# alv-around/mini-stark

Hardware: AMD Instinct MI355X
Metric: stark_proofs_per_s (higher is better)
Workload: dtype u64; 1 GPU; Fibonacci AIR, Goldilocks, 2^20 trace rows, blowup 8, 20 security bits (w=3, c=6, rounds=23, ood_queries=1, fri_queries=2); a step = 8 independent proofs in flight per GPU

## Files before the change

### mini-stark_amd/csrc/ctx.hpp

```cpp
#pragma once
#include "../../include/ministark.h"

#include <cstdarg>
#include <cstdio>
#include <cstdlib>
#include <map>
#include <new>
#include <string>
#include <type_traits>
#include <vector>

#include "field.hpp"
#include "merkle.hpp"
#include "ntt.hpp"
#include "poly.hpp"

namespace msctx {

struct DevBuf {
  void* p = nullptr; size_t cap = 0;
  int ensure(size_t bytes) {
    if (bytes <= cap) return 0;
    if (p) msrt::free_dev(p);
    p = nullptr; cap = 0;
// ... 251 lines not shown
  int finish_sharded_tree(TreeShape& ts, DevBuf& nodes, size_t Mloc);
  template <int EL>
  int tree_build_sharded_contiguous(const T* base, size_t col_stride, size_t row_stride, size_t limb_stride, u32 width, TreeShape& ts, DevBuf& nodes);
  int read_root(const DevBuf& nodes, const TreeShape& ts, u8* root);

  size_t N = 0, w = 0, L = 0, blowup = 0;
  int npolys = 0; size_t polys_cap = 0;
  struct Lin { std::vector<u64> s; std::vector<int> idx; };
  std::vector<Lin> poly_lin;
  std::vector<char> poly_mat; int lazy_lin = 1;
  void expand(int i, T scale, std::map<int, T>& acc) const {
    const Lin& li = poly_lin[i];
    if (li.idx.empty()) { auto it = acc.find(i); if (it == acc.end()) acc[i] = scale; else it->second = F::add(it->second, scale); return; }
    for (size_t t = 0; t < li.idx.size(); t++) expand(li.idx[t], F::mul(scale, F::from_u64(li.s[t] % F::P)), acc);
  }
  int materialize(int i);
  bool have_trace = false, have_polys = false, have_lde = false, have_validity = false;
  DevBuf d_trace[2], d_polys, d_coef, d_lde, d_trace_nodes, d_lde_nodes, d_io, d_partials, d_small;
  TreeShape trace_ts, lde_ts;
  size_t lde_c = 0;

  struct Round { DevBuf poly, cw, nodes; size_t cap = 0, ncoef = 0, D = 0; TreeShape ts; size_t m = 0;
                 bool dist = false, local_store = false; size_t S = 0;
                 bool base_cw = false;  };
  size_t shard_gather_chunk = 0;
  int shard_dist = 1;
  int proof_root_only = 0;
  const T* lpoly(const Round* r) const { return r->local_store ? r->poly.template as<T>() : r->poly.template as<T>() + (size_t)sh_rank * r->S; }
  size_t lstride(const Round* r) const { return r->local_store ? r->S : r->cap; }
  size_t lcount(const Round* r, size_t n) const { const size_t lo = (size_t)sh_rank * r->S; return n <= lo ? 0 : (n - lo < r->S ? n - lo : r->S); }
  size_t dist_chunk(size_t D) const {
    if (!sh_on || !shard_dist || !fri_blowup || !shardable(D / 2)) return 0;
    const size_t den = fri_blowup * (size_t)sh_world;
    if (D % den) return 0;
    const size_t S = D / den;
    return (S >= 2 && !(S & 1)) ? S : 0;
  }
  DevBuf d_carry, d_lq, d_pack, d_fullpoly;
  std::vector<Round*> rounds; size_t nrounds_done = 0, fri_rounds = 0, fri_blowup = 0;
  bool have_deep = false; XE cur_z; XE cur_B[2];
  DevBuf d_folded, d_sh, d_blob, d_tabs, d_targets, d_idx, d_deg, d_ovf;
  size_t blob_size = 0;

  int ensure_polys(size_t count);

  int init(int dev, u32 flags);
  ~Ctx() {
// ... 89 lines not shown
  template <int EC>
  int eval_views(const T* base, size_t poly_stride, size_t limb_stride, size_t kstride, const size_t* off, const size_t* count, int npoly, const XE& z, T* dst);
  template <int EC, int ITEMS>
  int eval_views_i(const T* base, size_t poly_stride, size_t limb_stride, size_t kstride, const size_t* off, const size_t* count, int npoly, const XE& z, T* dst, size_t maxc);
  static bool load_ext(const u64* v, XE* out) { for (int l = 0; l < E; l++) { if (v[l] >= F::P) return false; out->c[l] = F::from_u64(v[l]); } return true; }

  int shard_combine_launch(size_t off, size_t rank_stride, u32 n, const XE& zstep, T* out);
  bool dist_eval() const { return sh_on && shard_dist && N >= shard_min_leaves && N >= (size_t)sh_world * 2; }
  std::vector<int> eval_set() const { std::vector<int> ev; for (int i = 0; i < npolys; i++) if (poly_mat[i]) ev.push_back(i); ev.push_back(npolys); return ev; }
  int eval_finish(int q, const std::vector<int>& ev, u64* out);
  int eval_ext_sharded(const u64* z, int q, u64* out);

  int eval_ext(const u64* z, int q, u64* out) override;

  Round* round_slot(size_t i) { while (rounds.size() <= i) rounds.push_back(new Round()); return rounds[i]; }
  int round_commit(Round* r, size_t ncoef_in, int nonzero_limbs = E, const Round* prev = nullptr, const XE* alpha = nullptr);
  int degree_launch(const T* poly, size_t limb_stride, size_t n, unsigned long long** dres_out);
  int read_degree_and_root(const T* poly, size_t limb_stride, size_t n, Round* r, size_t* ncoef, u8* root);
  int fri_begin(size_t blowup_, size_t nrounds, u8* root0) override;
  int fri_deep(const u64* z, u64* B) override;

  typedef mspoly::SHJob<F, E> SHJ;
  typedef mspoly::SuffixHornerKernel<F, E> SHK;
  struct SHPlan { int nl; std::vector<SHJ> agg; std::vector<SHJ> fin; bool has_top_agg = false; SHJ top_agg; size_t P = 0; bool dist = false; };
  static size_t sh_scratch_elems(size_t m) {
    const size_t BS = mspoly::SH_BS;
    size_t tot = 0, cur = m;
    for (;;) { size_t nb = cur ? (cur + BS - 1) / BS : 1; tot += 2 * nb * E; if (nb <= 1) break; cur = nb; }
    return tot;
  }
  SHPlan sh_plan(const T* in, size_t in_limb_stride, size_t in_off, size_t in_stride, size_t m, const XE& z,
                 void* out, bool out_u64, size_t out_limb_stride, size_t out_off, size_t out_stride, T* h0, T* scratch,
                 const T* ext_carry = nullptr, T* top_agg = nullptr, bool out_h0 = false);
  static XE carry_scale(const XE& z, size_t m, size_t P) { return e_pow<F, E>(e_inv<F>(z), (u64)(P - m)); }
  int sh_launch_inline(const SHJ& j, int final_mode);
  int sh_launch_table(const SHJ* d_jobs, size_t njobs, size_t maxnb, int final_mode);
  int shard_carry_table(const mspoly::CarryJob<F, E>* d_jobs, size_t njobs);
  int suffix_horner(const T* in, size_t in_limb_stride, size_t in_off, size_t in_stride, size_t m, const XE& z,
                    T* out, size_t out_limb_stride, size_t out_off, size_t out_stride, T* h0);

  int gather_poly(const T* local, size_t S, size_t count, T* dst, size_t dst_stride);
  int fold_dist(Round* pr, Round* nr, const XE& a, size_t* nq_coef_out);
  int fri_fold_commit(const u64* alpha, u8* root) override;
  size_t fri_tail_max = (size_t)1 << 15;
  int fri_overlap = 0;
  msrt::Stream* side_stream = nullptr; msrt::Event* ev_side = nullptr; bool side_pending = false;
  struct StreamScope { Ctx* c; msrt::Stream* keep; StreamScope(Ctx* c_, msrt::Stream* s) : c(c_), keep(c_->stream) { c->stream = s; } ~StreamScope() { c->stream = keep; } };
  int join_side() { if (side_pending) { side_pending = false; CK(msrt::stream_wait_event(stream, ev_side)); } return 0; }
  int fri_tail_round(Round* pr, Round* nr, const XE& a, bool* done);
  template <class DG> int fri_tail_round_t(Round* pr, Round* nr, const XE& a, bool* done);
  int fri_round_info(int r, u64* ncoef, u64* D) override;
  int fri_round_poly_read(int r, u64* out) override;
  int fri_round_codeword_read(int r, u64* out) override;

  bool blob_external = false;
  int fri_query(const u64* betas, int nq, u8* ext_out, size_t ext_cap, size_t* ext_len) override;
  struct QueryPlan {
    typedef mspoly::CarryJob<F, E> CJ; typedef mspoly::FindJob<F, E> FJ; typedef msmerkle::PathJob<F, E> PJ; typedef msmerkle::ShardPathJob<F, E> SPJ;
    size_t W = 0; int nq = 0; size_t pos = 0; u8* blob = nullptr;
    T* d_h0 = nullptr; T* d_tg = nullptr; unsigned long long* d_ix = nullptr;
    std::vector<size_t> rec_off, path_off; std::vector<u64> qlen; std::vector<T> x1h;
    std::vector<std::vector<SHJ>> tables; std::vector<int> table_mode, table_part; size_t n_agg_tables = 0;
    std::vector<CJ> carry_jobs; bool any_dist = false;
    std::vector<msmerkle::CopyJob> unp; std::vector<size_t> unp_first, unp_cnt, chunk_c0, chunk_len;
    std::vector<FJ> fjobs; std::vector<PJ> pjobs; std::vector<SPJ> sjobs; std::vector<msmerkle::CopyJob> cjobs; size_t stage_bytes = 0;
    std::vector<size_t> toff; size_t off_f = 0, off_p = 0, off_sp = 0, off_cj = 0, off_rec = 0, off_ql = 0, off_x1 = 0, off_cr = 0, off_un = 0; const u8* dt = nullptr;
  };
  int query_layout(QueryPlan& q, int nq);
  int query_build(QueryPlan& q, const u64* betas);
  int query_scans(QueryPlan& q);
  int query_shard_assembly(QueryPlan& q);
  int query_openings(QueryPlan& q);
  size_t fri_proof_size() const override { return blob_size; }
  int fri_proof_read(u8* out) override;
  msrt::Stream* copy_stream = nullptr; msrt::Event* ev_blob = nullptr; msrt::Event* ev_copy = nullptr; bool copy_pending = false;
  int readback_sdma = 2, sdma_gpu = -1, sdma_state = 0 , last_io_engine = 0;
  msrt::Sdma::Signal sdma_sig{0}, sdma_up_sig{0}; bool sdma_pending = false; int upload_sdma = 1;
  u8* readback_dst = nullptr; size_t readback_bytes = 0;
  double sdma_timeout_s = 20.0;
  bool sdma_ready();
  int poison(const char* what);
  int io_engine() const override { return last_io_engine; }
  int fri_proof_read_async(u8* out) override;
  int fri_proof_wait() override;
  struct Upload { const u64* src = nullptr; size_t N = 0, w = 0; int slot = 0; bool pending = false; } up;
  int trace_slot = 0;
  int trace_upload_async(const u64* trace, size_t N_, size_t w_) override;
  int trace_to_device(const u64* trace, const u64** dsrc);
  int upload_wait(const char* what);

  int merkle_commit(const u64* leafs, size_t leaf_num, int ext, size_t lpn, size_t ic, u8* nodes_out, size_t cap, size_t* nn, u8* root) override;
  template <int EL>
  int merkle_prove_t(const u64* leafs, size_t leaf_num, size_t lpn, const u64* leaf, u8* out, size_t cap, size_t* len);
// ... 10 lines not shown
```

### mini-stark_amd/csrc/fri_commit.cpp

```cpp
#include "ctx.hpp"
#include "fri_tail.hpp"

namespace msctx {

template <class F>
int Ctx<F>::round_commit(Round* r, size_t ncoef_in, int nonzero_limbs, const Round* prev, const XE* alpha) {
  if (ctz64(r->D) > F::TWO_ADICITY) return fail(MS_ERR_SHAPE, "FRI domain larger than the field's two-adicity");
  RQ(tree_shape(r->D, 2, 2, &r->ts));
  r->m = 0;
  r->base_cw = false;
  {
    const bool shard_next = shardable(r->D / 2);
    bool z_outside_base = false;
    for (int l = 1; l < E; l++) z_outside_base = z_outside_base || cur_z.c[l] != 0;
    if (prev && fri_pointwise && z_outside_base && prev->D == 2 * r->D && prev->ts.sharded == shard_next) {
      Plan* pl;
      RQ(get_plan(ctz64(prev->D), 0, false, &pl));
      const size_t W = (size_t)sh_world;
      const size_t m_out = shard_next ? r->D / (2 * W) : r->D;
      const size_t local = shard_next ? 2 * m_out : r->D;
      if (shard_next) r->m = m_out;
      if (r->cw.ensure(local * E * sizeof(T))) return fail(MS_ERR_NOMEM, "codeword");
      const size_t total = m_out * (shard_next ? 2 : 1);
      const XE c = e_add<F, E>(cur_B[0], e_mul<F>(cur_B[1], *alpha));
// ... 101 lines not shown

template <class F>
int Ctx<F>::fri_begin(size_t blowup_, size_t nrounds, u8* root0) {
  if (!have_validity) return fail(MS_ERR_STATE, "fri_begin before mix");
  if (!root0 || nrounds < 1 || !blowup_) return fail(MS_ERR_ARG, "fri_begin");
  nrounds_done = 0; have_deep = false; blob_size = 0;
  fri_rounds = nrounds; fri_blowup = blowup_;
  if (!d_deg.p && d_deg.ensure(256)) return fail(MS_ERR_NOMEM, "degree word");
  CK(msrt::memset_dev(d_deg.p, 0, 256, stream));
  Round* r = round_slot(0);
  const size_t VL = validity_len;
  r->cap = VL;
  if (r->poly.ensure(VL * E * sizeof(T))) return fail(MS_ERR_NOMEM, "round poly");
  CK(msrt::memset_dev(r->poly.p, 0, VL * E * sizeof(T), stream));
  CK(msrt::d2d(r->poly.p, d_polys.as<T>() + (size_t)npolys * N, VL * sizeof(T), stream));
  size_t nc;
  if (validity_len_host) nc = validity_ncoef;
  else RQ(read_degree_and_root(r->poly.template as<T>(), r->cap, VL, nullptr, &nc, nullptr));
  r->ncoef = nc;
  const size_t deg = nc ? nc - 1 : 0;
  size_t dsize = (deg + 1) * blowup_;
  size_t D = 1; while (D < dsize) D <<= 1;
  r->D = D;
  r->S = dist_chunk(D); r->dist = r->S != 0; r->local_store = false;
  RQ(round_commit(r, nc, 1));
  RQ(read_root(r->nodes, r->ts, root0));
  nrounds_done = 1;
  return MS_OK;
}

template <class F>
int Ctx<F>::fri_deep(const u64* z, u64* B) {
  if (nrounds_done == 0 || nrounds_done >= fri_rounds) return fail(MS_ERR_STATE, "fri_deep out of order");
  if (!z || !B) return fail(MS_ERR_ARG, "fri_deep");
  if (!load_ext(z, &cur_z)) return fail(MS_ERR_ARG, "z not canonical");
  Round* r = rounds[nrounds_done - 1];
  size_t off[2] = {0, 1}, cnt[2] = {(r->ncoef + 1) / 2, r->ncoef / 2};
  T* dst = reinterpret_cast<T*>(pinned);
  if (r->dist) {
    const size_t lc = lcount(r, r->ncoef);
    cnt[0] = (lc + 1) / 2; cnt[1] = lc / 2;
    { PartScope part(this); RQ((eval_views<E>(lpoly(r), 0, lstride(r), 2, off, cnt, 2, cur_z, reinterpret_cast<T*>(xs)))); }
    RQ(exchange(MS_XCHG_ALL_GATHER, 2 * E * sizeof(T)));
    RQ(shard_combine_launch(0, 2 * E, 2, e_pow<F, E>(cur_z, (u64)(r->S / 2)), dst));
  } else
  { arm_next_eval = true; RQ((eval_views<E>(r->poly.template as<T>(), 0, r->cap, 2, off, cnt, 2, cur_z, dst))); }
// ... 138 lines not shown
  }
  *nq_coef_out = nq_coef;
  return 0;
}

template <class F>
int Ctx<F>::fri_tail_round(Round* pr, Round* nr, const XE& a, bool* done) {
  if (digest == MS_DIGEST_KECCAK256) return fri_tail_round_t<msmerkle::Keccak256Kernels>(pr, nr, a, done);
  if (digest == MS_DIGEST_SHA3_256) return fri_tail_round_t<msmerkle::Sha3_256Kernels>(pr, nr, a, done);
  if (digest == MS_DIGEST_BLAKE3) return fri_tail_round_t<msmerkle::Blake3Kernels>(pr, nr, a, done);
  return digest == MS_DIGEST_BLAKE2S256 ? fri_tail_round_t<msmerkle::Blake2sKernels>(pr, nr, a, done) : fri_tail_round_t<msmerkle::Sha256Kernels>(pr, nr, a, done);
}
template <class F> template <class DG>
int Ctx<F>::fri_tail_round_t(Round* pr, Round* nr, const XE& a, bool* done) {
  *done = false;
  const size_t n = pr->ncoef, m = (n + 1) / 2, Dn = nr->D, M = Dn / 2;
  bool z_outside_base = false;
  for (int l = 1; l < E; l++) z_outside_base = z_outside_base || cur_z.c[l] != 0;
  if (!fri_tail_max || pr->D > fri_tail_max || pr->dist || pr->ts.sharded || shardable(M) || !fri_pointwise || !z_outside_base || m > (size_t)mspoly::SH_BS || M < 1) return 0;
  typedef msfri::FriTailKernel<F, E, DG> TK;
  if (M > (size_t)TK::WG_GROUPS << TK::TreeK::MAX_LEVELS) return 0;
  if (ctz64(Dn) > F::TWO_ADICITY) return fail(MS_ERR_SHAPE, "FRI domain larger than the field's two-adicity");
  RQ(tree_shape(Dn, 2, 2, &nr->ts));
  nr->m = 0; nr->base_cw = false;
  if (nr->poly.ensure(nr->cap * E * sizeof(T)) || d_folded.ensure((m + 1) * E * sizeof(T)) || nr->cw.ensure(Dn * E * sizeof(T)) || nr->nodes.ensure(nr->ts.nodes * 32) ||
      d_sh.ensure(sh_scratch_elems(m) * sizeof(T)))
    return fail(MS_ERR_NOMEM, "fused FRI round");
  Plan* pl;
  RQ(get_plan(ctz64(pr->D), 0, false, &pl));
  typename TK::Params tp;
  memset(&tp, 0, sizeof tp);
  tp.do_coef = m >= 2 ? 1 : 0;
  tp.fold = typename TK::FoldK::Params{pr->poly.template as<T>(), pr->cap, n, d_folded.as<T>(), m, a, nullptr};
  if (tp.do_coef) {
    SHPlan sp = sh_plan(d_folded.as<T>(), m, 0, 1, m, cur_z, nr->poly.template as<T>(), false, nr->cap, 0, 1, nullptr, d_sh.as<T>());
    if (sp.nl != 1) return fail(MS_ERR_STATE, "fused FRI round: scan of more than one block");
    tp.scan.jobs = nullptr; tp.scan.inline_job = sp.fin[0]; tp.scan.final_mode = 1;
  }
  unsigned long long* dres = d_deg.as<unsigned long long>();
  tp.deg = typename TK::DegK::Params{nr->poly.template as<T>(), nr->cap, m >= 2 ? m - 1 : 0, dres, 0};
  const size_t per = M < (size_t)TK::WG_GROUPS ? M : (size_t)TK::WG_GROUPS, G = M / per;
  tp.G = (u32)G;
  const XE c = e_add<F, E>(cur_B[0], e_mul<F>(cur_B[1], a));
  tp.eval.src = pr->cw.template as<T>(); tp.eval.src_limb_stride = pr->D; tp.eval.dst = nr->cw.template as<T>(); tp.eval.dst_limb_stride = Dn;
  tp.eval.m_out = Dn; tp.eval.log_m = (u32)ctz64(Dn); tp.eval.groups = 1; tp.eval.shard_W = 0; tp.eval.shard_k = 0;
  tp.eval.tw_lo = pl->tw_lo.template as<T>(); tp.eval.tw_hi = pl->tw_hi.template as<T>(); tp.eval.lo_bits = (u32)pl->lo_bits; tp.eval.log_D = (u32)ctz64(pr->D);
  tp.eval.alpha = a; tp.eval.c2 = e_add<F, E>(c, c); tp.eval.z = cur_z; tp.eval.inv2 = f_inv<F>(F::from_u64(2));
// ... 125 lines not shown
```

### mini-stark_amd/csrc/fri_query.cpp

```cpp
#include "ctx.hpp"

namespace msctx {


template <class F>
int Ctx<F>::query_layout(QueryPlan& q, int nq) {
  const size_t W = fri_rounds - 1;
  q.W = W; q.nq = nq;
  q.rec_off.assign(W * nq, 0); q.path_off.assign(W * nq * 2, 0); q.qlen.assign(W ? W : 1, 0);
  size_t pos = 0;
  for (size_t i = 0; i < W; i++) {
    Round* pr = rounds[i];
    if (pr->D / 2 != rounds[i + 1]->D) return fail(MS_ERR_SHAPE, "round domains do not halve (fri.rs:134-137)");
    q.qlen[i] = pr->ncoef >= 3 ? pr->ncoef - 2 : 0;
    const size_t nlev = pr->ts.levels - 1;
    const size_t path_bytes = 8 + 2 * E * 8 + 8 + nlev * 2 * 32;
    for (int j = 0; j < nq; j++) {
      q.rec_off[i * nq + j] = pos;
      pos += 6 * E * 8 + 8 + q.qlen[i] * E * 8;
      q.path_off[(i * nq + j) * 2] = pos; pos += path_bytes;
      q.path_off[(i * nq + j) * 2 + 1] = pos; pos += path_bytes;
    }
  }
  q.pos = pos;
// ... 13 lines not shown
  for (size_t i = 0; i < W; i++) {
    Round* pr = rounds[i];
    if (!pr->dist) continue;
    const size_t Sh = pr->S / 2;
    for (size_t r = 0; r < Wr; r++) for (int j = 0; j < nq; j++) {
      const size_t lo_h = r * Sh, hi_h = lo_h + Sh, q_ = q.qlen[i];
      size_t t1 = 2 * (hi_h - 1); if (t1 > q_) t1 = q_;
      size_t t0 = 2 * ((lo_h > 1 ? lo_h : 1) - 1); if (t0 > t1) t0 = t1;
      const size_t k = (r * W + i) * nq + j;
      sl_t0[k] = t0; sl_len[k] = t1 - t0; sl_off[k] = sl_tot[r]; sl_tot[r] += (t1 - t0) * E * 8;
    }
  }
  size_t pack_max = 0;
  for (size_t r = 0; r < Wr; r++) if (sl_tot[r] > pack_max) pack_max = sl_tot[r];
  if (q.any_dist && (d_pack.ensure(pack_max + 64) || d_carry.ensure(((W + 1) * nq * 2 + 1) * E * sizeof(T)))) return fail(MS_ERR_NOMEM, "query slices");
  if (q.any_dist && ((W + 1) * nq * 2 * E * sizeof(T) * Wr > xcap || xcap / Wr < 4096)) return fail(MS_ERR_NOMEM, "exchange buffers too small for the query phase");
  {
    std::vector<SHPlan> shplans;
    T* scr = d_sh.as<T>();
    for (size_t i = 0; i <= W; i++) {
      Round* pr = rounds[i];
      const T gp = f_root_of_unity<F>(ctz64(pr->D));
      const size_t n = pr->ncoef, mm[2] = {(n + 1) / 2, n / 2};
      for (int j = 0; j < nq; j++) {
        u64 beta = betas[j];
        if (i < W) { if (beta > pr->D) beta %= pr->D; }
        else beta %= pr->D;
        const T x1 = f_pow<F>(gp, beta);
        q.x1h[i * nq + j] = x1;
        const XE X3 = e_from_base<F, E>(F::mul(x1, x1));
        for (int sgn = 0; sgn < 2; sgn++) {
          void* out = nullptr;
          T* h0 = d_h0 + ((i * nq + j) * 2 + sgn) * E;
          if (pr->dist) {
            const size_t Sh = pr->S / 2, lo_h = (size_t)sh_rank * Sh, cl = mm[sgn] <= lo_h ? 0 : (mm[sgn] - lo_h < Sh ? mm[sgn] - lo_h : Sh);
            const size_t qi = q.carry_jobs.size();
            T* slot_carry = d_carry.as<T>() + qi * E;
            size_t out_off = 0;
            if (i < W) {
              const size_t k = ((size_t)sh_rank * W + i) * nq + j;
              out = reinterpret_cast<u64*>(d_pack.as<u8>() + sl_off[k]) - sl_t0[k] * E;
              out_off = (size_t)sgn * E + lo_h * 2 * E;
            }
            CJ cj; memset(&cj, 0, sizeof cj);
            cj.agg_off = (u32)(qi * E); cj.has_first = 0; cj.zA = e_one<F, E>(); cj.zB = e_pow<F, E>(X3, (u64)Sh);
            cj.carry_out = slot_carry; cj.tail_out = nullptr; cj.h0_out = h0; cj.scale = e_zero<F, E>();
            if (cl) {
              SHPlan pl = sh_plan(lpoly(pr), lstride(pr), sgn, 2, cl, X3, out, true, 1, out_off, 2 * E, nullptr, scr, slot_carry, reinterpret_cast<T*>(xs) + qi * E, sh_rank > 0);
              cj.scale = carry_scale(X3, cl, pl.P);
              pl.dist = true;
              shplans.push_back(pl);
              scr += sh_scratch_elems(cl);
            }
            q.carry_jobs.push_back(cj);
            continue;
          }
          if (i < W) out = blob + q.rec_off[i * nq + j] + (6 * E + 1) * 8;
          shplans.push_back(sh_plan(pr->poly.template as<T>(), pr->cap, sgn, 2, mm[sgn], X3, out, true, 1, (size_t)sgn * E, 2 * E, h0, scr));
          scr += sh_scratch_elems(mm[sgn]);
        }
      }
    }
    int max_nl = 1;
    for (auto& pl : shplans) if (pl.nl > max_nl) max_nl = pl.nl;
    auto add = [&](std::vector<SHJ>& t, int mode, bool part) { if (!t.empty()) { q.tables.push_back(t); q.table_mode.push_back(mode); q.table_part.push_back(part ? 1 : 0); } };
    for (int nl = 1; nl <= max_nl; nl++) {
      for (int l = 0; l + 1 < nl; l++) { std::vector<SHJ> t; bool ad = true; for (auto& pl : shplans) if (pl.nl == nl) { t.push_back(pl.agg[l]); ad = ad && pl.dist; } add(t, 0, ad); }
      { std::vector<SHJ> t; for (auto& pl : shplans) if (pl.nl == nl && pl.has_top_agg) t.push_back(pl.top_agg); add(t, 0, true); }
    }
    q.n_agg_tables = q.tables.size();
    for (int nl = 1; nl <= max_nl; nl++)
      for (int l = nl - 1; l >= 0; l--) { std::vector<SHJ> t; bool ad = true; for (auto& pl : shplans) if (pl.nl == nl) { t.push_back(pl.fin[l]); ad = ad && pl.dist; } add(t, 1, ad); }
  }
  if (q.any_dist && pack_max) {
    size_t Cb = (pack_max < ((xcap / Wr) & ~(size_t)63)) ? pack_max : ((xcap / Wr) & ~(size_t)63);
    if (shard_gather_chunk && shard_gather_chunk < Cb) Cb = shard_gather_chunk;
    for (size_t c0 = 0; c0 < pack_max; c0 += Cb) {
      const size_t len = pack_max - c0 < Cb ? pack_max - c0 : Cb;
      q.chunk_c0.push_back(c0); q.chunk_len.push_back(len); q.unp_first.push_back(q.unp.size());
      for (size_t r = 0; r < Wr; r++) for (size_t i = 0; i < W; i++) for (int j = 0; j < nq; j++) {
        const size_t k = (r * W + i) * nq + j, b0 = sl_off[k], b1 = b0 + sl_len[k] * E * 8;
        const size_t p0 = b0 > c0 ? b0 : c0, p1 = b1 < c0 + len ? b1 : c0 + len;
        if (p0 >= p1) continue;
        q.unp.push_back(msmerkle::CopyJob{xr + r * len + (p0 - c0), blob + q.rec_off[i * nq + j] + (6 * E + 1) * 8 + sl_t0[k] * E * 8 + (p0 - b0), p1 - p0});
      }
      q.unp_cnt.push_back(q.unp.size() - q.unp_first.back());
    }
  }
  typedef typename QueryPlan::FJ FJ;
  typedef typename QueryPlan::PJ PJ;
  typedef typename QueryPlan::SPJ SPJ;
  const bool shard = sh_on;
  q.fjobs.resize(W);
  q.stage_bytes = 0;
  for (size_t i = 0; i < W; i++) {
// ... 7 lines not shown
      u8* out = dst;
      if (shard) { out = xs + q.stage_bytes; q.cjobs.push_back(msmerkle::CopyJob{out, dst, path_bytes}); q.stage_bytes += path_bytes; }
      if (pr->ts.sharded)
        q.sjobs.push_back(SPJ{pr->cw.template as<T>(), 2 * pr->m, pr->m, pr->nodes.template as<u32>(), pr->nodes.template as<u32>() + (2 * pr->ts.Mloc - 1) * 8, pr->ts.Mloc,
                              2, (u32)sh_world, (u32)sh_rank, (u32)nlev, d_ix + i * 2 * nq + t, out});
      else if (!shard || sh_rank == 0)
        q.pjobs.push_back(PJ{pr->cw.template as<T>(), pr->D, pr->nodes.template as<u32>(), pr->D, 2, 2, (u32)nlev, d_ix + i * 2 * nq + t, out});
    }
  }
  if (shard && (q.stage_bytes > xcap || W * nq * 2 * 8 > xcap)) return fail(MS_ERR_NOMEM, "exchange buffers too small for the query phase");
  size_t bytes = 0;
  q.toff.assign(q.tables.size(), 0);
  for (size_t k = 0; k < q.tables.size(); k++) { q.toff[k] = bytes; bytes += q.tables[k].size() * sizeof(SHJ); }
  q.off_f = bytes; bytes += q.fjobs.size() * sizeof(FJ);
  q.off_p = bytes; bytes += q.pjobs.size() * sizeof(PJ);
  q.off_sp = bytes; bytes += q.sjobs.size() * sizeof(SPJ);
  q.off_cj = bytes; bytes += q.cjobs.size() * sizeof(msmerkle::CopyJob);
  q.off_rec = bytes; bytes += q.rec_off.size() * sizeof(size_t);
  q.off_ql = bytes; bytes += q.qlen.size() * 8;
  q.off_x1 = bytes; bytes += q.x1h.size() * sizeof(T);
  bytes = (bytes + 15) & ~(size_t)15;
  q.off_cr = bytes; bytes += q.carry_jobs.size() * sizeof(CJ);
  q.off_un = bytes; bytes += q.unp.size() * sizeof(msmerkle::CopyJob);
  u8* tab;
  RQ(tabs_host(bytes + 8, &tab));
  for (size_t k = 0; k < q.tables.size(); k++) memcpy(tab + q.toff[k], q.tables[k].data(), q.tables[k].size() * sizeof(SHJ));
  if (!q.fjobs.empty()) memcpy(tab + q.off_f, q.fjobs.data(), q.fjobs.size() * sizeof(FJ));
  if (!q.pjobs.empty()) memcpy(tab + q.off_p, q.pjobs.data(), q.pjobs.size() * sizeof(PJ));
  if (!q.sjobs.empty()) memcpy(tab + q.off_sp, q.sjobs.data(), q.sjobs.size() * sizeof(SPJ));
  if (!q.cjobs.empty()) memcpy(tab + q.off_cj, q.cjobs.data(), q.cjobs.size() * sizeof(msmerkle::CopyJob));
  if (!q.rec_off.empty()) memcpy(tab + q.off_rec, q.rec_off.data(), q.rec_off.size() * sizeof(size_t));
  memcpy(tab + q.off_ql, q.qlen.data(), q.qlen.size() * 8);
  memcpy(tab + q.off_x1, q.x1h.data(), q.x1h.size() * sizeof(T));
  if (!q.carry_jobs.empty()) memcpy(tab + q.off_cr, q.carry_jobs.data(), q.carry_jobs.size() * sizeof(CJ));
  if (!q.unp.empty()) memcpy(tab + q.off_un, q.unp.data(), q.unp.size() * sizeof(msmerkle::CopyJob));
  if (d_tabs.ensure(bytes + 8)) return fail(MS_ERR_NOMEM, "query tables");
  CK(msrt::h2d(d_tabs.p, tab, bytes + 8, stream));
  q.dt = d_tabs.as<u8>();
  return 0;
}

template <class F>
int Ctx<F>::query_scans(QueryPlan& q) {
  typedef typename QueryPlan::CJ CJ;
  const size_t ncarry = q.carry_jobs.size();
  auto carries = [&]() -> int {
    RQ(exchange(MS_XCHG_ALL_GATHER, ncarry * E * sizeof(T)));
    return shard_carry_table(reinterpret_cast<const CJ*>(q.dt + q.off_cr), ncarry);
  };
  if (ncarry) CK(msrt::memset_dev(xs, 0, ncarry * E * sizeof(T), stream));
  for (size_t k = 0; k < q.tables.size(); k++) {
    if (k == q.n_agg_tables && ncarry) RQ(carries());
    size_t maxnb = 1;
    for (auto& j : q.tables[k]) { size_t nb = j.m ? (j.m + mspoly::SH_BS - 1) / mspoly::SH_BS : 1; if (nb > maxnb) maxnb = nb; }
    PartScopeIf part(this, q.table_part[k] != 0);
    RQ(sh_launch_table(reinterpret_cast<const SHJ*>(q.dt + q.toff[k]), q.tables[k].size(), maxnb, q.table_mode[k]));
  }
  if (q.n_agg_tables == q.tables.size() && ncarry) RQ(carries());
  return 0;
}

template <class F>
int Ctx<F>::query_shard_assembly(QueryPlan& q) {
  for (size_t c = 0; c < q.chunk_c0.size(); c++) {
    CK(msrt::d2d(xs, d_pack.as<u8>() + q.chunk_c0[c], q.chunk_len[c], stream));
    RQ(exchange(proof_root_only ? MS_XCHG_GATHER : MS_XCHG_ALL_GATHER, q.chunk_len[c]));
    if (q.unp_cnt[c] && (!proof_root_only || sh_rank == 0)) {
      size_t maxw = 1;
      for (size_t u = 0; u < q.unp_cnt[c]; u++) { const size_t wgs = (q.unp[q.unp_first[c] + u].bytes / 8 + msmerkle::CopyRangesKernel::WORDS - 1) / msmerkle::CopyRangesKernel::WORDS; if (wgs > maxw) maxw = wgs; }
      msmerkle::CopyRangesKernel::Params up{reinterpret_cast<const msmerkle::CopyJob*>(q.dt + q.off_un) + q.unp_first[c], (u32)q.unp_cnt[c]};
      CK(run<msmerkle::CopyRangesKernel>(K_IO, (unsigned)maxw, (unsigned)q.unp_cnt[c], msmerkle::CopyRangesKernel::THREADS, 0, up));
    }
  }
  return 0;
}

template <class F>
int Ctx<F>::query_openings(QueryPlan& q) {
  typedef typename QueryPlan::FJ FJ;
  typedef typename QueryPlan::PJ PJ;
  typedef typename QueryPlan::SPJ SPJ;
// ... 111 lines not shown
    if (!e) e = msrt::d2h(pinned, base + off_ix, 8, stream);
    if (!e) e = msrt::d2h(out, base + off_path, plen, stream);
    if (!e) e = msrt::sync(stream);
    if (e) rc = fail_rt(e, "merkle_prove");
    else if (*reinterpret_cast<unsigned long long*>(pinned) == ~0ULL) rc = fail(MS_ERR_LEAF_NOT_FOUND, "leaf is not included in the tree");
  }
  msrt::sync(stream);
  ds.release(); dn.release(); dw.release();
  return rc;
}

template <class F>
int Ctx<F>::merkle_prove(const u64* leafs, size_t leaf_num, int ext, size_t lpn, const u64* leaf, u8* out, size_t cap, size_t* len) {
  if (!leafs || !leaf) return fail(MS_ERR_ARG, "null argument");
  if (ext == 1) return merkle_prove_t<1>(leafs, leaf_num, lpn, leaf, out, cap, len);
  if (ext == E) return merkle_prove_t<E>(leafs, leaf_num, lpn, leaf, out, cap, len);
  return fail(MS_ERR_ARG, "ext must be 1 or the field's extension degree");
}

#define MS_INSTANTIATE(FF) \
  template int Ctx<FF>::query_layout(Ctx<FF>::QueryPlan& q, int nq); \
  template int Ctx<FF>::query_build(Ctx<FF>::QueryPlan& q, const u64* betas); \
  template int Ctx<FF>::query_scans(Ctx<FF>::QueryPlan& q); \
  template int Ctx<FF>::query_shard_assembly(Ctx<FF>::QueryPlan& q); \
  template int Ctx<FF>::query_openings(Ctx<FF>::QueryPlan& q); \
  template int Ctx<FF>::fri_query(const u64* betas, int nq, u8* ext_out, size_t ext_cap, size_t* ext_len); \
  template int Ctx<FF>::merkle_prove(const u64* leafs, size_t leaf_num, int ext, size_t lpn, const u64* leaf, u8* out, size_t cap, size_t* len);
MS_INSTANTIATE(GL)
MS_INSTANTIATE(BB)
#undef MS_INSTANTIATE

}
```

### mini-stark_amd/csrc/poly.hpp

```cpp
#pragma once
#include "field.hpp"
#include "ntt.hpp"

namespace mspoly {

constexpr int THREADS = 256;

template <class F> struct TransposeInKernel {
  typedef typename F::T T;
  static constexpr int THREADS = mspoly::THREADS;
  struct Params { const u64* src; T* dst; size_t N, w, dst_stride; T rinv; int mont;  u32* bad; };
  static MS_HD int nphases(const Params&) { return 1; }
  static MS_DEV void phase(int, const Params& p, int bx, int, int tid, int nthreads, unsigned char*) {
    const size_t f = (size_t)bx * nthreads + tid;
    if (f >= p.N * p.w) return;
    const size_t row = f / p.w, col = f - row * p.w;
    const u64 raw = p.src[f];
    const bool oob = raw >= F::P;
    if (oob && p.bad) *p.bad = 1;
    T v = F::from_u64(oob ? 0 : raw);
    if (p.mont) v = F::mul(v, p.rinv);
    p.dst[col * p.dst_stride + row] = v;
  }
};
// ... 362 lines not shown
      const size_t j = j0 + i;
      if (j >= jb.m && !(j == 0)) continue;
      for (int l = 0; l < E; l++) {
        const T v = fbuf[(size_t)l * SH_BS + i];
        if (j == 0) {
          if (jb.h0) jb.h0[l] = v;
          if (jb.out_h0 && jb.out) {
            const size_t o = (size_t)l * jb.out_limb_stride + jb.out_off - jb.out_stride;
            if (jb.out_u64) reinterpret_cast<u64*>(jb.out)[o] = F::to_u64(v); else reinterpret_cast<T*>(jb.out)[o] = v;
          }
        } else if (jb.out) {
          const size_t o = (size_t)l * jb.out_limb_stride + jb.out_off + (j - 1) * jb.out_stride;
          if (jb.out_u64) reinterpret_cast<u64*>(jb.out)[o] = F::to_u64(v); else reinterpret_cast<T*>(jb.out)[o] = v;
        }
      }
      if (jb.tail_zero && jb.out && j + 1 == jb.m) {
        for (int l = 0; l < E; l++) {
          T tv = 0;
          if (jb.tail_zero == 2) tv = (i + 1 < SH_BS) ? fbuf[(size_t)l * SH_BS + i + 1] : sc[(size_t)l * (THREADS + 1) + THREADS];
          const size_t o = (size_t)l * jb.out_limb_stride + jb.out_off + j * jb.out_stride;
          if (jb.out_u64) reinterpret_cast<u64*>(jb.out)[o] = F::to_u64(tv); else reinterpret_cast<T*>(jb.out)[o] = tv;
        }
      }
    }
  }
};

template <class F> MS_HD typename F::T fold_base_inv(typename F::T x) { return f_inv<F>(x); }
template <> MS_HD u64 fold_base_inv<GL>(u64 x) { return gl_inv_chain(x); }
template <class F, int E, int ITEMS_ = 8> struct FriFoldEvalKernel {
  typedef typename F::T T;
  typedef Ext<F, E> X;
  static_assert(E == 2 || E == 4, "quadratic or quartic tower");
  static constexpr int THREADS = mspoly::THREADS;
  static constexpr int ITEMS = ITEMS_;
  struct Params {
    const T* src; size_t src_limb_stride; T* dst; size_t dst_limb_stride;
    size_t m_out; u32 log_m , groups, shard_W, shard_k;
    const T* tw_lo; const T* tw_hi; u32 lo_bits, log_D;
    X alpha, c2 , z;
    T inv2;
  };
  static MS_HD int nphases(const Params&) { return 1; }
  static MS_DEV T w_tab(const Params& p, size_t e) {
    T tw = p.tw_lo[e & (((size_t)1 << p.lo_bits) - 1)];
    const size_t eh = e >> p.lo_bits;
// ... 568 lines not shown
```

### mini-stark_amd/csrc/session.cpp

```cpp
#include "ctx.hpp"
#include "running.hpp"

namespace msctx {

template <class F>
int Ctx<F>::profile_end(char* out, size_t cap) {
  static const char* names[K_COUNT] = {"ntt_pass", "scale_pow", "leaf_hash", "inner_hash", "transpose_in", "io_copy", "lincomb", "mix", "eval", "eval_reduce",
                                       "fold", "suffix_horner", "degree", "find_first", "merkle_path", "query_points", "fri_tail", "mix_terms", "mix_air", "air_inv", "aux_running"};
  msrt::sync(stream);
  double ms[K_COUNT] = {0}, by[K_COUNT] = {0}, ms_part = 0, ms_repl = 0, repl_by[K_COUNT] = {0}; unsigned long long cnt[K_COUNT] = {0};
  std::map<int, double> sub_ms, sub_by; std::map<int, unsigned long long> sub_cnt;
  for (auto& r : prof_recs) {
    float t = 0.f; msrt::event_elapsed_ms(&t, r.a, r.b);
    ms[r.kid] += t; by[r.kid] += r.bytes; cnt[r.kid]++;
    if (r.part) ms_part += t; else { ms_repl += t; repl_by[r.kid] += t; }
    if (r.kid == K_NTT_PASS) { sub_ms[r.sub] += t; sub_by[r.sub] += r.bytes; sub_cnt[r.sub]++; }
    msrt::event_destroy(r.a); msrt::event_destroy(r.b);
  }
  prof_recs.clear(); prof_on = false;
  std::string j = "{";
  for (int k = 0; k < K_COUNT; k++) {
    char buf[256];
    snprintf(buf, sizeof buf, "%s\"%s\": {\"launches\": %llu, \"ms\": %.6f, \"alg_bytes\": %.0f}", k ? ", " : "", names[k], cnt[k], ms[k], by[k]);
    j += buf;
// ... 61 lines not shown
  d_polys.release();
  d_polys = nb; polys_cap = ncap;
  return 0;
}

template <class F>
int Ctx<F>::init(int dev, u32 flags) {
  device = dev; zae = (flags & MS_FLAG_ZERO_DISPLAY_EMPTY) ? 1 : 0; trace_mont = (flags & MS_FLAG_TRACE_MONT64) ? 1 : 0; fri_overlap = (flags & MS_FLAG_LATENCY) ? 1 : 0; poll_sync = fri_overlap;
  if ((flags & MS_FLAG_DIGEST_BLAKE2S) && (flags & MS_FLAG_DIGEST_BLAKE3)) return fail(MS_ERR_ARG, "ms_create: MS_FLAG_DIGEST_BLAKE2S and MS_FLAG_DIGEST_BLAKE3 exclude each other");
  { const u32 d = flags & (MS_FLAG_DIGEST_BLAKE2S | MS_FLAG_DIGEST_BLAKE3 | MS_FLAG_DIGEST_KECCAK256 | MS_FLAG_DIGEST_SHA3_256); if (d & (d - 1)) return fail(MS_ERR_ARG, "ms_create: the MS_FLAG_DIGEST_* flags exclude each other"); }
  digest = (flags & MS_FLAG_DIGEST_KECCAK256) ? MS_DIGEST_KECCAK256 : (flags & MS_FLAG_DIGEST_SHA3_256) ? MS_DIGEST_SHA3_256
         : (flags & MS_FLAG_DIGEST_BLAKE3) ? MS_DIGEST_BLAKE3 : (flags & MS_FLAG_DIGEST_BLAKE2S) ? MS_DIGEST_BLAKE2S256 : MS_DIGEST_SHA256;
  if (const char* e = getenv("MS_NTT_KMAX")) { int v = atoi(e); if (v >= 5 && v <= msntt::MAX_LOG_R) ntt_kmax = v; }
  if (const char* e = getenv("MS_NTT_FAST")) ntt_fast = atoi(e);
  if (const char* e = getenv("MS_NTT_V2")) ntt_v2 = atoi(e);
  if (const char* e = getenv("MS_NTT_V2_REGPASS")) ntt_v2_regpass = atoi(e);
  if (const char* e = getenv("MS_NTT_SHARE")) ntt_share = atoi(e);
  if (const char* e = getenv("MS_NTT_COOP_WGS")) { int v = atoi(e); if (v >= 8 && v <= 65536) ntt_coop_wgs = v & ~7; }
  if (const char* e = getenv("MS_LDE_LINEAR")) lde_linear = atoi(e);
  if (const char* e = getenv("MS_LAZY_LINCOMB")) lazy_lin = atoi(e);
  if (const char* e = getenv("MS_LDE_MULTI")) lde_multi = atoi(e);
  if (const char* e = getenv("MS_LDE_VIRTUAL")) lde_virtual = atoi(e);
  if (const char* e = getenv("MS_FRI_POINTWISE")) fri_pointwise = atoi(e);
  if (const char* e = getenv("MS_FOLD_SMALL_MAX")) fold_small_max = (size_t)atol(e);
  if (const char* e = getenv("MS_FRI_TAIL_MAX")) fri_tail_max = (size_t)atol(e);
  if (const char* e = getenv("MS_FRI_OVERLAP")) fri_overlap = atoi(e);
  if (const char* e = getenv("MS_SYNC_POLL")) poll_sync = atoi(e);
  if (const char* e = getenv("MS_EVAL_SMALL_MAX")) eval_small_max = (size_t)atol(e);
  if (const char* e = getenv("MS_TREE_SUBTREE_PARENTS")) subtree_parents = (size_t)atol(e);
  if (const char* e = getenv("MS_AUX_TILE")) { const int v = atoi(e); if (v >= msrun::THREADS && v <= AUX_TILE_DEFAULT && !(v & (v - 1))) aux_tile = v; }
  if (const char* e = getenv("MS_UPLOAD")) upload_sdma = !strcmp(e, "hip") ? 0 : 1;
  if (const char* e = getenv("MS_SDMA_TIMEOUT_S")) { const double v = atof(e); if (v > 0) sdma_timeout_s = v; }
  if (const char* e = getenv("MS_READBACK")) readback_sdma = !strcmp(e, "hip") ? 0 : (!strcmp(e, "sdma-async") ? 1 : 2);
  if (const char* e = getenv("MS_LEAF_LAZY_MIN")) leaf_lazy_min = atoi(e);
  if (const char* e = getenv("MS_TREE_TOP")) { int v = atoi(e); if (v >= 1 && v <= 65536) tree_top_parents = v; }
  if (const char* e = getenv("MS_SHARD_MIN_LEAVES")) { long v = atol(e); if (v >= 1) shard_min_leaves = (size_t)v; }
  if (const char* e = getenv("MS_SHARD_DIST")) shard_dist = atoi(e);
  if (const char* e = getenv("MS_SHARD_WORLD1")) allow_w1 = atoi(e);
  if (const char* e = getenv("MS_SHARD_STUB")) shard_stub = atoi(e);
  if (const char* e = getenv("MS_SHARD_GATHER_CHUNK")) { long v = atol(e); if (v >= 64) shard_gather_chunk = (size_t)v & ~(size_t)63; }
  if (const char* e = getenv("MS_SHARD_SLICES")) { int v = atoi(e); if (v >= 1 && v <= 64) { shard_slices = v; shard_slices_set = true; } }
  if (const char* e = getenv("MS_SHARD_SLICE_MIN")) { long v = atol(e); if (v >= 1) shard_slice_min = (size_t)v; }
  if (const char* e = getenv("MS_RCCL_MAX_PIECE")) { long long v = atoll(e); if (v >= 64 && v <= ((long long)1 << 30)) rccl_max_piece = (size_t)v & ~(size_t)63; }
  CK(msrt::set_device(dev));
  CK(msrt::stream_create(&own_stream));
  stream = own_stream;
// ... 246 lines not shown
```

Measured before the change: 280.9 proofs/s.

## Add tiled query-scan kernel fusing even/odd suffix-Horner passes per FRI round

Adds a QueryScanKernel that loads each coefficient tile once and computes suffix-Horner aggregates and final outputs for both even and odd halves and up to two queries at a time. It uses precomputed power tables and wave-level scans. The level-0 aggregate and final jobs of non-distributed rounds move out of the generic SH tables into this kernel, with a base-field variant for the first round's polynomial. The aim is to cut redundant coefficient reads and kernel launches in the FRI query phase, at the cost of more complex LDS indexing and new correctness risk.

```diff
diff --git a/mini-stark_amd/csrc/ctx.hpp b/mini-stark_amd/csrc/ctx.hpp
--- a/mini-stark_amd/csrc/ctx.hpp
+++ b/mini-stark_amd/csrc/ctx.hpp
@@ -297,7 +297,8 @@
 
   struct Round { DevBuf poly, cw, nodes; size_t cap = 0, ncoef = 0, D = 0; TreeShape ts; size_t m = 0;
                  bool dist = false, local_store = false; size_t S = 0;
-                 bool base_cw = false;  };
+                 bool base_cw = false;
+                 bool base_poly = false;  };
   size_t shard_gather_chunk = 0;
   int shard_dist = 1;
   int proof_root_only = 0;
@@ -433,7 +434,8 @@
 
   typedef mspoly::SHJob<F, E> SHJ;
   typedef mspoly::SuffixHornerKernel<F, E> SHK;
-  struct SHPlan { int nl; std::vector<SHJ> agg; std::vector<SHJ> fin; bool has_top_agg = false; SHJ top_agg; size_t P = 0; bool dist = false; };
+  struct SHPlan { int nl; std::vector<SHJ> agg; std::vector<SHJ> fin; bool has_top_agg = false; SHJ top_agg; size_t P = 0; bool dist = false;
+                  bool tile = false;  };
   static size_t sh_scratch_elems(size_t m) {
     const size_t BS = mspoly::SH_BS;
     size_t tot = 0, cur = m;
@@ -472,6 +474,8 @@
     T* d_h0 = nullptr; T* d_tg = nullptr; unsigned long long* d_ix = nullptr;
     std::vector<size_t> rec_off, path_off; std::vector<u64> qlen; std::vector<T> x1h;
     std::vector<std::vector<SHJ>> tables; std::vector<int> table_mode, table_part; size_t n_agg_tables = 0;
+    typedef mspoly::QSJob<F, E> QSJ;
+    std::vector<QSJ> qs[4]; size_t qs_tiles[4] = {0, 0, 0, 0}, off_qs[4] = {0, 0, 0, 0};
     std::vector<CJ> carry_jobs; bool any_dist = false;
     std::vector<msmerkle::CopyJob> unp; std::vector<size_t> unp_first, unp_cnt, chunk_c0, chunk_len;
     std::vector<FJ> fjobs; std::vector<PJ> pjobs; std::vector<SPJ> sjobs; std::vector<msmerkle::CopyJob> cjobs; size_t stage_bytes = 0;
@@ -480,6 +484,8 @@
   int query_layout(QueryPlan& q, int nq);
   int query_build(QueryPlan& q, const u64* betas);
   int query_scans(QueryPlan& q);
+  int query_scan = 1;
+  int qs_launch(QueryPlan& q, int k);
   int query_shard_assembly(QueryPlan& q);
   int query_openings(QueryPlan& q);
   size_t fri_proof_size() const override { return blob_size; }
diff --git a/mini-stark_amd/csrc/fri_commit.cpp b/mini-stark_amd/csrc/fri_commit.cpp
--- a/mini-stark_amd/csrc/fri_commit.cpp
+++ b/mini-stark_amd/csrc/fri_commit.cpp
@@ -147,6 +147,7 @@
   size_t dsize = (deg + 1) * blowup_;
   size_t D = 1; while (D < dsize) D <<= 1;
   r->D = D;
+  r->base_poly = true;
   r->S = dist_chunk(D); r->dist = r->S != 0; r->local_store = false;
   RQ(round_commit(r, nc, 1));
   RQ(read_root(r->nodes, r->ts, root0));
@@ -331,7 +332,7 @@
   if (M > (size_t)TK::WG_GROUPS << TK::TreeK::MAX_LEVELS) return 0;
   if (ctz64(Dn) > F::TWO_ADICITY) return fail(MS_ERR_SHAPE, "FRI domain larger than the field's two-adicity");
   RQ(tree_shape(Dn, 2, 2, &nr->ts));
-  nr->m = 0; nr->base_cw = false;
+  nr->m = 0; nr->base_cw = false; nr->base_poly = false;
   if (nr->poly.ensure(nr->cap * E * sizeof(T)) || d_folded.ensure((m + 1) * E * sizeof(T)) || nr->cw.ensure(Dn * E * sizeof(T)) || nr->nodes.ensure(nr->ts.nodes * 32) ||
       d_sh.ensure(sh_scratch_elems(m) * sizeof(T)))
     return fail(MS_ERR_NOMEM, "fused FRI round");
diff --git a/mini-stark_amd/csrc/fri_query.cpp b/mini-stark_amd/csrc/fri_query.cpp
--- a/mini-stark_amd/csrc/fri_query.cpp
+++ b/mini-stark_amd/csrc/fri_query.cpp
@@ -59,6 +59,9 @@
       Round* pr = rounds[i];
       const T gp = f_root_of_unity<F>(ctz64(pr->D));
       const size_t n = pr->ncoef, mm[2] = {(n + 1) / 2, n / 2};
+      const bool tiled = query_scan && !pr->dist;
+      const size_t first_plan = shplans.size();
+      std::vector<T> x3s((size_t)nq);
       for (int j = 0; j < nq; j++) {
         u64 beta = betas[j];
         if (i < W) { if (beta > pr->D) beta %= pr->D; }
@@ -66,6 +69,7 @@
         const T x1 = f_pow<F>(gp, beta);
         q.x1h[i * nq + j] = x1;
         const XE X3 = e_from_base<F, E>(F::mul(x1, x1));
+        x3s[j] = X3.c[0];
         for (int sgn = 0; sgn < 2; sgn++) {
           void* out = nullptr;
           T* h0 = d_h0 + ((i * nq + j) * 2 + sgn) * E;
@@ -94,20 +98,57 @@
           }
           if (i < W) out = blob + q.rec_off[i * nq + j] + (6 * E + 1) * 8;
           shplans.push_back(sh_plan(pr->poly.template as<T>(), pr->cap, sgn, 2, mm[sgn], X3, out, true, 1, (size_t)sgn * E, 2 * E, h0, scr));
+          shplans.back().tile = tiled;
           scr += sh_scratch_elems(mm[sgn]);
         }
+      }
+      if (!tiled) continue;
+      typedef typename QueryPlan::QSJ QSJ;
+      const size_t BS = mspoly::QS_BS;
+      const int SEG = mspoly::SH_SEG;
+      for (int g0 = 0; g0 < nq; g0 += mspoly::QS_NQ) {
+        QSJ fj; memset(&fj, 0, sizeof fj);
+        fj.in = pr->poly.template as<T>(); fj.in_limb_stride = pr->cap; fj.n = n;
+        for (int s = 0; s < 2; s++) fj.nb[s] = mm[s] ? (mm[s] + BS - 1) / BS : 1;
+        fj.nq = (u32)(nq - g0 < mspoly::QS_NQ ? nq - g0 : mspoly::QS_NQ);
+        QSJ aj = fj;
+        bool any_agg = false;
+        for (u32 k = 0; k < fj.nq; k++) {
+          const int j = g0 + (int)k;
+          const T z = x3s[j], z8 = f_pow<F>(z, (u64)SEG), zi8 = f_inv<F>(z8);
+          const T z128 = f_pow<F>(z8, 16), zi128 = f_pow<F>(zi8, 16);
+          T a = F::from_u64(1), b = F::from_u64(1), c = zi8, d = F::from_u64(1);
+          for (int t = 0; t < 16; t++) {
+            fj.tab[k][t] = a; fj.tab[k][16 + t] = b; fj.tab[k][32 + t] = c; fj.tab[k][48 + t] = d;
+            a = F::mul(a, z8); b = F::mul(b, z128); c = F::mul(c, zi8); d = F::mul(d, zi128);
+          }
+          fj.z[k] = z; fj.zbs[k] = f_pow<F>(z, (u64)BS);
+          memcpy(aj.tab[k], fj.tab[k], sizeof fj.tab[k]); aj.z[k] = z; aj.zbs[k] = fj.zbs[k];
+          if (i < W) fj.out[k] = reinterpret_cast<u64*>(blob + q.rec_off[i * nq + j] + (6 * E + 1) * 8);
+          fj.h0[k] = d_h0 + ((i * nq + j) * 2) * E;
+          for (int s = 0; s < 2; s++) {
+            const SHPlan& pl = shplans[first_plan + (size_t)2 * j + s];
+            fj.carry[k][s] = pl.fin[0].carry;
+            if (pl.nl > 1) { aj.agg[k][s] = pl.agg[0].agg; any_agg = true; }
+          }
+        }
+        fj.ntiles = (u32)(i < W ? fj.nb[0] : 1);
+        aj.ntiles = (u32)aj.nb[0];
+        const int v = pr->base_poly ? 0 : 1;
+        if (any_agg) { q.qs[v].push_back(aj); if (aj.ntiles > q.qs_tiles[v]) q.qs_tiles[v] = aj.ntiles; }
+        q.qs[2 + v].push_back(fj); if (fj.ntiles > q.qs_tiles[2 + v]) q.qs_tiles[2 + v] = fj.ntiles;
       }
     }
     int max_nl = 1;
     for (auto& pl : shplans) if (pl.nl > max_nl) max_nl = pl.nl;
     auto add = [&](std::vector<SHJ>& t, int mode, bool part) { if (!t.empty()) { q.tables.push_back(t); q.table_mode.push_back(mode); q.table_part.push_back(part ? 1 : 0); } };
     for (int nl = 1; nl <= max_nl; nl++) {
-      for (int l = 0; l + 1 < nl; l++) { std::vector<SHJ> t; bool ad = true; for (auto& pl : shplans) if (pl.nl == nl) { t.push_back(pl.agg[l]); ad = ad && pl.dist; } add(t, 0, ad); }
+      for (int l = 0; l + 1 < nl; l++) { std::vector<SHJ> t; bool ad = true; for (auto& pl : shplans) if (pl.nl == nl && !(l == 0 && pl.tile)) { t.push_back(pl.agg[l]); ad = ad && pl.dist; } add(t, 0, ad); }
       { std::vector<SHJ> t; for (auto& pl : shplans) if (pl.nl == nl && pl.has_top_agg) t.push_back(pl.top_agg); add(t, 0, true); }
     }
     q.n_agg_tables = q.tables.size();
     for (int nl = 1; nl <= max_nl; nl++)
-      for (int l = nl - 1; l >= 0; l--) { std::vector<SHJ> t; bool ad = true; for (auto& pl : shplans) if (pl.nl == nl) { t.push_back(pl.fin[l]); ad = ad && pl.dist; } add(t, 1, ad); }
+      for (int l = nl - 1; l >= 0; l--) { std::vector<SHJ> t; bool ad = true; for (auto& pl : shplans) if (pl.nl == nl && !(l == 0 && pl.tile)) { t.push_back(pl.fin[l]); ad = ad && pl.dist; } add(t, 1, ad); }
   }
   if (q.any_dist && pack_max) {
     size_t Cb = (pack_max < ((xcap / Wr) & ~(size_t)63)) ? pack_max : ((xcap / Wr) & ~(size_t)63);
@@ -161,6 +202,8 @@
   bytes = (bytes + 15) & ~(size_t)15;
   q.off_cr = bytes; bytes += q.carry_jobs.size() * sizeof(CJ);
   q.off_un = bytes; bytes += q.unp.size() * sizeof(msmerkle::CopyJob);
+  bytes = (bytes + 15) & ~(size_t)15;
+  for (int k = 0; k < 4; k++) { q.off_qs[k] = bytes; bytes += q.qs[k].size() * sizeof(typename QueryPlan::QSJ); }
   u8* tab;
   RQ(tabs_host(bytes + 8, &tab));
   for (size_t k = 0; k < q.tables.size(); k++) memcpy(tab + q.toff[k], q.tables[k].data(), q.tables[k].size() * sizeof(SHJ));
@@ -173,6 +216,7 @@
   memcpy(tab + q.off_x1, q.x1h.data(), q.x1h.size() * sizeof(T));
   if (!q.carry_jobs.empty()) memcpy(tab + q.off_cr, q.carry_jobs.data(), q.carry_jobs.size() * sizeof(CJ));
   if (!q.unp.empty()) memcpy(tab + q.off_un, q.unp.data(), q.unp.size() * sizeof(msmerkle::CopyJob));
+  for (int k = 0; k < 4; k++) if (!q.qs[k].empty()) memcpy(tab + q.off_qs[k], q.qs[k].data(), q.qs[k].size() * sizeof(typename QueryPlan::QSJ));
   if (d_tabs.ensure(bytes + 8)) return fail(MS_ERR_NOMEM, "query tables");
   CK(msrt::h2d(d_tabs.p, tab, bytes + 8, stream));
   q.dt = d_tabs.as<u8>();
@@ -188,6 +232,7 @@
     return shard_carry_table(reinterpret_cast<const CJ*>(q.dt + q.off_cr), ncarry);
   };
   if (ncarry) CK(msrt::memset_dev(xs, 0, ncarry * E * sizeof(T), stream));
+  RQ(qs_launch(q, 0)); RQ(qs_launch(q, 1));
   for (size_t k = 0; k < q.tables.size(); k++) {
     if (k == q.n_agg_tables && ncarry) RQ(carries());
     size_t maxnb = 1;
@@ -196,6 +241,20 @@
     RQ(sh_launch_table(reinterpret_cast<const SHJ*>(q.dt + q.toff[k]), q.tables[k].size(), maxnb, q.table_mode[k]));
   }
   if (q.n_agg_tables == q.tables.size() && ncarry) RQ(carries());
+  RQ(qs_launch(q, 2)); RQ(qs_launch(q, 3));
+  return 0;
+}
+
+template <class F>
+int Ctx<F>::qs_launch(QueryPlan& q, int k) {
+  if (q.qs[k].empty()) return 0;
+  typedef typename QueryPlan::QSJ QSJ;
+  auto go = [&](auto* kernel) {
+    typedef typename std::remove_pointer<decltype(kernel)>::type QK;
+    typename QK::Params p; p.jobs = reinterpret_cast<const QSJ*>(q.dt + q.off_qs[k]); p.final_mode = k >= 2;
+    return run_coop<QK>(K_SUFFIX_HORNER, (unsigned)q.qs_tiles[k], QK::THREADS, QK::lds_bytes(), p, (unsigned)q.qs[k].size());
+  };
+  if (k & 1) CK(go((mspoly::QueryScanKernel<F, E, E>*)nullptr)); else CK(go((mspoly::QueryScanKernel<F, E, 1>*)nullptr));
   return 0;
 }
 
@@ -353,6 +412,7 @@
   template int Ctx<FF>::query_layout(Ctx<FF>::QueryPlan& q, int nq); \
   template int Ctx<FF>::query_build(Ctx<FF>::QueryPlan& q, const u64* betas); \
   template int Ctx<FF>::query_scans(Ctx<FF>::QueryPlan& q); \
+  template int Ctx<FF>::qs_launch(Ctx<FF>::QueryPlan& q, int k); \
   template int Ctx<FF>::query_shard_assembly(Ctx<FF>::QueryPlan& q); \
   template int Ctx<FF>::query_openings(Ctx<FF>::QueryPlan& q); \
   template int Ctx<FF>::fri_query(const u64* betas, int nq, u8* ext_out, size_t ext_cap, size_t* ext_len); \
diff --git a/mini-stark_amd/csrc/poly.hpp b/mini-stark_amd/csrc/poly.hpp
--- a/mini-stark_amd/csrc/poly.hpp
+++ b/mini-stark_amd/csrc/poly.hpp
@@ -408,6 +408,149 @@
           if (jb.out_u64) reinterpret_cast<u64*>(jb.out)[o] = F::to_u64(tv); else reinterpret_cast<T*>(jb.out)[o] = tv;
         }
       }
+    }
+  }
+};
+
+constexpr int QS_NQ = 2;
+constexpr int QS_BS = SH_BS;
+template <class F, int E> struct QSJob {
+  typedef typename F::T T;
+  const T* in; size_t in_limb_stride, n;
+  size_t nb[2];
+  u64* out[QS_NQ];
+  T* h0[QS_NQ];
+  T* agg[QS_NQ][2];
+  const T* carry[QS_NQ][2];
+  T z[QS_NQ], zbs[QS_NQ];
+  T tab[QS_NQ][64];
+  u32 nq, ntiles;
+};
+template <class F, int E, int EC> struct QueryScanKernel {
+  typedef typename F::T T;
+  typedef QSJob<F, E> Job;
+  static_assert(EC == 1 || EC == E, "base-field or full coefficients");
+  static constexpr int THREADS = mspoly::THREADS, SEG = SH_SEG, NW = THREADS / 64;
+  static constexpr int TILE = 2 * QS_BS;
+  static constexpr int PTILE = TILE + TILE / 16;
+  static constexpr int RUN = 2 * SEG * EC;
+  struct Params { const Job* jobs; int final_mode; };
+  static MS_HD size_t lds_bytes() { return ((size_t)EC * PTILE + (size_t)QS_NQ * 2 * EC * NW) * sizeof(T); }
+  static MS_DEV void run(const Params& p, int bx, int by, int, int tid, unsigned char* lds) {
+    const Job& jb = p.jobs[by];
+    if ((u32)bx >= jb.ntiles) return;
+    T* buf = reinterpret_cast<T*>(lds);
+    T* red = buf + (size_t)EC * PTILE;
+    const size_t k0 = (size_t)bx * TILE, j0 = (size_t)bx * QS_BS;
+    const size_t mm[2] = {(jb.n + 1) / 2, jb.n / 2};
+    const int lane = tid & 63, wave = tid >> 6;
+    for (int i = tid; i < TILE; i += THREADS) {
+      const size_t k = k0 + i;
+#pragma unroll
+      for (int l = 0; l < EC; l++) buf[(size_t)l * PTILE + i + (i >> 4)] = (k < jb.n) ? jb.in[(size_t)l * jb.in_limb_stride + k] : (T)0;
+    }
+    msrt::wg_barrier();
+    T c[2][SEG][EC];
+#pragma unroll
+    for (int i = 0; i < SEG; i++)
+#pragma unroll
+      for (int s = 0; s < 2; s++)
+#pragma unroll
+        for (int l = 0; l < EC; l++) c[s][i][l] = buf[(size_t)l * PTILE + 17 * tid + 2 * i + s];
+    msrt::wg_barrier();
+    T b[QS_NQ][2][EC];
+    for (int q = 0; q < QS_NQ; q++) {
+      const bool live = (u32)q < jb.nq;
+      const T z = live ? F::tw_of(jb.z[q]) : (T)0;
+      const T pw = live ? F::tw_of(F::mul(jb.tab[q][tid & 15], jb.tab[q][16 + (tid >> 4)])) : (T)0;
+#pragma unroll
+      for (int s = 0; s < 2; s++) {
+        T a[EC];
+#pragma unroll
+        for (int l = 0; l < EC; l++) a[l] = c[s][SEG - 1][l];
+#pragma unroll
+        for (int i = SEG - 2; i >= 0; i--)
+#pragma unroll
+          for (int l = 0; l < EC; l++) a[l] = F::add(F::mul_tw(a[l], z), c[s][i][l]);
+#pragma unroll
+        for (int l = 0; l < EC; l++) b[q][s][l] = F::mul_tw(a[l], pw);
+      }
+    }
+    if (!p.final_mode) {
+#pragma unroll
+      for (int q = 0; q < QS_NQ; q++)
+#pragma unroll
+        for (int s = 0; s < 2; s++)
+#pragma unroll
+          for (int l = 0; l < EC; l++) {
+            T v = b[q][s][l];
+#pragma unroll
+            for (int m = 32; m >= 1; m >>= 1) v = F::add(v, (T)msrt::wave_shfl_xor((unsigned long long)v, m));
+            if (lane == 0) red[(size_t)((q * 2 + s) * EC + l) * NW + wave] = v;
+          }
+      msrt::wg_barrier();
+      if (tid < QS_NQ * 2 * E) {
+        const int q = tid / (2 * E), s = (tid / E) & 1, l = tid % E;
+        if ((u32)q < jb.nq && jb.agg[q][s] && (size_t)bx < jb.nb[s]) {
+          T v = 0;
+          if (l < EC) for (int w = 0; w < NW; w++) v = F::add(v, red[(size_t)((q * 2 + s) * EC + l) * NW + w]);
+          jb.agg[q][s][(size_t)l * jb.nb[s] + bx] = v;
+        }
+      }
+      return;
+    }
+    T ex[QS_NQ][2][EC];
+#pragma unroll
+    for (int q = 0; q < QS_NQ; q++)
+#pragma unroll
+      for (int s = 0; s < 2; s++)
+#pragma unroll
+        for (int l = 0; l < EC; l++) {
+          T sc = b[q][s][l], tot = sc;
+#pragma unroll
+          for (int d = 1; d < 64; d <<= 1) {
+            const T o = (T)msrt::wave_shfl_xor((unsigned long long)tot, d);
+            if (!(lane & d)) sc = F::add(sc, o);
+            tot = F::add(tot, o);
+          }
+          ex[q][s][l] = F::sub(sc, b[q][s][l]);
+          if (lane == 0) red[(size_t)((q * 2 + s) * EC + l) * NW + wave] = tot;
+        }
+    msrt::wg_barrier();
+    for (int q = 0; q < QS_NQ; q++) {
+      if ((u32)q >= jb.nq) break;
+      const T z = F::tw_of(jb.z[q]), zbs = F::tw_of(jb.zbs[q]);
+      const T ipw = F::tw_of(F::mul(jb.tab[q][32 + (tid & 15)], jb.tab[q][48 + (tid >> 4)]));
+#pragma unroll
+      for (int s = 0; s < 2; s++) {
+        const bool cin = jb.carry[q][s] && (size_t)bx < jb.nb[s];
+        T h[EC];
+#pragma unroll
+        for (int l = 0; l < EC; l++) {
+          T v = ex[q][s][l];
+          for (int w = wave + 1; w < NW; w++) v = F::add(v, red[(size_t)((q * 2 + s) * EC + l) * NW + w]);
+          if (cin) v = F::add(v, F::mul_tw(jb.carry[q][s][(size_t)l * jb.nb[s] + bx], zbs));
+          h[l] = F::mul_tw(v, ipw);
+        }
+#pragma unroll
+        for (int i = SEG - 1; i >= 0; i--)
+#pragma unroll
+          for (int l = 0; l < EC; l++) {
+            h[l] = F::add(F::mul_tw(h[l], z), c[s][i][l]);
+            buf[(size_t)((SEG * tid + i) * 2 + s) * EC + l + tid] = h[l];
+          }
+      }
+      msrt::wg_barrier();
+      for (int w = tid; w < QS_BS * 2 * E; w += THREADS) {
+        const int i = w / (2 * E), r = w % (2 * E), s = r / E, l = r % E;
+        const size_t j = j0 + i;
+        if (j && j >= mm[s]) continue;
+        T v = 0;
+        if (l < EC) { const int e = (i * 2 + s) * EC + l; v = buf[e + e / RUN]; }
+        if (j == 0) jb.h0[q][r] = v;
+        else if (jb.out[q]) jb.out[q][(j - 1) * (2 * E) + r] = F::to_u64(v);
+      }
+      msrt::wg_barrier();
     }
   }
 };
diff --git a/mini-stark_amd/csrc/session.cpp b/mini-stark_amd/csrc/session.cpp
--- a/mini-stark_amd/csrc/session.cpp
+++ b/mini-stark_amd/csrc/session.cpp
@@ -107,6 +107,7 @@
   if (const char* e = getenv("MS_LDE_MULTI")) lde_multi = atoi(e);
   if (const char* e = getenv("MS_LDE_VIRTUAL")) lde_virtual = atoi(e);
   if (const char* e = getenv("MS_FRI_POINTWISE")) fri_pointwise = atoi(e);
+  if (const char* e = getenv("MS_QUERY_SCAN")) query_scan = atoi(e);
   if (const char* e = getenv("MS_FOLD_SMALL_MAX")) fold_small_max = (size_t)atol(e);
   if (const char* e = getenv("MS_FRI_TAIL_MAX")) fri_tail_max = (size_t)atol(e);
   if (const char* e = getenv("MS_FRI_OVERLAP")) fri_overlap = atoi(e);
```

Result: no change. 283.1 proofs/s (median of 6 runs) (+0.8%).
